# CederGroupHub/smol

Measured on AMD Instinct MI355X. Metric: attempted MC flips/s (node) + ns/flip/replica, 4096-site FCC canonical, higher is better.
Workload: dtype f64

## Files before the change

smol_amd/csrc/mc_lean.h:

```cpp
#pragma once
#include "smolmc_common.h"

template <int CTRL> __device__ __forceinline__ double dpp_xor_add(double v) {
    const int lo = __builtin_amdgcn_update_dpp(__double2loint(v), __double2loint(v), CTRL, 0xf, 0xf, true);
    const int hi = __builtin_amdgcn_update_dpp(__double2hiint(v), __double2hiint(v), CTRL, 0xf, 0xf, true);
    return v + __hiloint2double(hi, lo);
}
__device__ __forceinline__ double wave_sum_all(double v) {
    v = dpp_xor_add<0xB1>(v);
    v = dpp_xor_add<0x4E>(v);
    v = dpp_xor_add<0x141>(v);
    v = dpp_xor_add<0x140>(v);
    {
        const unsigned lo = (unsigned)__double2loint(v), hi = (unsigned)__double2hiint(v);
        const auto a = __builtin_amdgcn_permlane16_swap(lo, lo, false, false);
        const auto b = __builtin_amdgcn_permlane16_swap(hi, hi, false, false);
        v = __hiloint2double((int)b[0], (int)a[0]) + __hiloint2double((int)b[1], (int)a[1]);
    }
    {
        const unsigned lo = (unsigned)__double2loint(v), hi = (unsigned)__double2hiint(v);
        const auto a = __builtin_amdgcn_permlane32_swap(lo, lo, false, false);
        const auto b = __builtin_amdgcn_permlane32_swap(hi, hi, false, false);
        v = __hiloint2double((int)b[0], (int)a[0]) + __hiloint2double((int)b[1], (int)a[1]);
    }
    return v;
}

template <int CTRL> __device__ __forceinline__ float dpp_add_f32(float v) {
    const int t = __builtin_amdgcn_update_dpp(0, __float_as_int(v), CTRL, 0xf, 0xf, true);
    return v + __int_as_float(t);
}
__device__ __forceinline__ float wave_sum_f32_uniform(float v) {
    v = dpp_add_f32<0xB1>(v);
    v = dpp_add_f32<0x4E>(v);
    v = dpp_add_f32<0x141>(v);
    v = dpp_add_f32<0x140>(v);
    float total;
    asm volatile("s_nop 1\n\t"
                 "v_add_f32_dpp %1, %1, %1 row_bcast:15 row_mask:0xa bank_mask:0xf\n\t"
                 "s_nop 1\n\t"
                 "v_add_f32_dpp %1, %1, %1 row_bcast:31 row_mask:0xc bank_mask:0xf\n\t"
                 "s_nop 1\n\t"
                 "v_readlane_b32 %0, %1, 63\n\t"
                 "s_nop 1"
                 : "=s"(total), "+v"(v));
    return total;
}


__device__ __forceinline__ double lean_ewald_partial(const LeanParams &P, const uint8_t *occ, int lane,
                                                     int s, int swa, int swm, int swb) {
    const double *g = P.ew_G + (size_t)s * P.ew_nact;
    const int W = P.ew_W, na = P.ew_nact;
    double out = 0;
    for (int j0 = lane; j0 < na; j0 += 64 * 8) {
        int k[8];
        double gk[8], q[8];
#pragma unroll
        for (int u = 0; u < 8; ++u) {
            const int jj = min(j0 + 64 * u, na - 1);
            k[u] = P.ew_act[jj];
            gk[u] = g[jj];
        }
#pragma unroll
        for (int u = 0; u < 8; ++u)
            q[u] = P.ew_qs[(size_t)k[u] * W + (int)occ[lean_swz(k[u], swa, swm, swb)]];
#pragma unroll
        for (int u = 0; u < 8; ++u)
            out = fma((j0 + 64 * u < na && k[u] != s) ? q[u] : 0.0, gk[u], out);
    }
    return out;
}

template <int FOOT = 2, bool PRE = false>
__device__ __forceinline__ void field_apply(const LeanParams &P, double *phi, int lane, int s, double dq,
                                            const uint32_t (&e0)[27], const bool have_e0) {
    const int js = s - P.sbase;
    const double keep = phi[js];
    const LeanParamsKernarg Q = rare_params();
    const unsigned char *gx = (const unsigned char *)Q->ew_gx;
    if (gx != nullptr) {
        const uint32_t *E8 = Q->ew_E8;
        const uint32_t s8[1] = {Q->ew_S8[js]};
        const double d[1] = {dq};
        if (PRE && have_e0) field_sweep_gx_pre27(phi, E8, gx, lane, P.ew_nact, s8, d, e0);
        else field_sweep_gx_multi<1, FOOT>(phi, E8, gx, lane, P.ew_nact, s8, d);
    } else {
        const double *g = P.ew_G + (size_t)s * P.ew_nact;
        field_sweep<false>(phi, g, g, lane, P.ew_nact, dq, 0.0);
    }
    phi[js] = keep;
}

template <int FOOT = 2>
__device__ __forceinline__ void field_apply(const LeanParams &P, double *phi, int lane, int s, double dq) {
    const uint32_t none[27] = {};
    field_apply<FOOT, false>(P, phi, lane, s, dq, none, false);
}

template <int FOOT = 1, bool FEW = false>
__device__ __forceinline__ void field_apply_flips(double *phi, int lane, int nfl, int vsite, double vdq) {
    const LeanParamsKernarg Q = rare_params();

    const unsigned char *gx = (const unsigned char *)Q->ew_gx;
    auto site_of = [&](int f) { return (int)rdlane((uint32_t)vsite, f); };
    auto dq_of = [&](int f) {
        return __hiloint2double((int)rdlane((uint32_t)__double2hiint(vdq), f), (int)rdlane((uint32_t)__double2loint(vdq), f));
    };
    const int sb = Q->sbase, na = Q->ew_nact;
    if (gx == nullptr) {
        const double *G = Q->ew_G;
        for (int f = 0; f < nfl; ++f) {
            const double dqf = dq_of(f);
            if (dqf == 0.0) continue;
            const double *g = G + (size_t)site_of(f) * na;
            field_sweep<false>(phi, g, g, lane, na, dqf, 0.0);
        }
        return;
    }
    const uint32_t *E8 = Q->ew_E8, *S8 = Q->ew_S8;
    for (int f0 = 0; f0 < nfl; f0 += 4) {
        const int n = min(4, nfl - f0);
        uint32_t s8[4];
        double dq[4];
#pragma unroll
        for (int k = 0; k < 4; ++k) {
            const int f = k < n ? f0 + k : f0;
            s8[k] = S8[site_of(f) - sb];
            dq[k] = k < n ? dq_of(f) : 0.0;
        }
        if (FEW && n <= 3) {
            const uint32_t a[3] = {s8[0], s8[1], s8[2]};
            const double d[3] = {dq[0], dq[1], dq[2]};
            field_sweep_gx_multi<3, FOOT>(phi, E8, gx, lane, na, a, d);
        } else if (n == 1) {
            const uint32_t a[1] = {s8[0]};
            const double d[1] = {dq[0]};
            field_sweep_gx_multi<1, FOOT>(phi, E8, gx, lane, na, a, d);
        } else if (n == 2) {
            const uint32_t a[2] = {s8[0], s8[1]};
            const double d[2] = {dq[0], dq[1]};
            field_sweep_gx_multi<2, FOOT>(phi, E8, gx, lane, na, a, d);
        } else if (n == 3) {
            const uint32_t a[3] = {s8[0], s8[1], s8[2]};
            const double d[3] = {dq[0], dq[1], dq[2]};
            field_sweep_gx_multi<3, FOOT>(phi, E8, gx, lane, na, a, d);
        } else {
            field_sweep_gx_multi<4, FOOT>(phi, E8, gx, lane, na, s8, dq);
        }
    }
}

template <int FOOT = 1>
__device__ __forceinline__ void field_apply2(const LeanParams &P, double *phi, int lane, int s1, double dq1,
                                             int s2, double dq2) {
    const int j1 = s1 - P.sbase, j2 = s2 - P.sbase;
    const LeanParamsKernarg Q = rare_params();
    const unsigned char *gx = (const unsigned char *)Q->ew_gx;
    if (gx != nullptr) {
        const uint32_t *E8 = Q->ew_E8, *S8 = Q->ew_S8;
        const uint32_t s8[2] = {S8[j1], S8[j2]};
        const double d[2] = {dq1, dq2};
        field_sweep_gx_multi<2, FOOT>(phi, E8, gx, lane, P.ew_nact, s8, d);
        return;
    }
    const double *g1 = P.ew_G + (size_t)s1 * P.ew_nact, *g2 = P.ew_G + (size_t)s2 * P.ew_nact;
    const double keep1 = phi[j1], keep2 = phi[j2];
    const double c12 = g2[j1], c21 = g1[j2];
    field_sweep<true>(phi, g1, g2, lane, P.ew_nact, dq1, dq2);
    if (j1 != j2) {
        phi[j1] = fma(dq2, c12, keep1);
        phi[j2] = fma(dq1, c21, keep2);
    } else {
        phi[j1] = keep1;
    }
}

__device__ __forceinline__ uint32_t bounded(uint32_t a, uint32_t lim) {
#ifdef SMOLMC_BOUNDS
    if (a >= lim) __builtin_trap();
#else
    (void)lim;
#endif
    return a;
}

template <int NW> struct RowWords { uint32_t w[NW]; };
template <int NW>
__device__ __forceinline__ RowWords<NW> load_row(__amdgpu_buffer_rsrc_t rs, uint32_t voff, uint32_t soff) {
    RowWords<NW> r;
    if constexpr (NW == 2) {
        const auto v = __builtin_amdgcn_raw_buffer_load_b64(rs, voff, soff, 0);
        r.w[0] = v[0]; r.w[1] = v[1];
    } else if constexpr (NW == 3) {
        const auto v = __builtin_amdgcn_raw_buffer_load_b96(rs, voff, soff, 0);
        r.w[0] = v[0]; r.w[1] = v[1]; r.w[2] = v[2];
    } else if constexpr (NW == 4) {
        const auto v = __builtin_amdgcn_raw_buffer_load_b128(rs, voff, soff, 0);
        r.w[0] = v[0]; r.w[1] = v[1]; r.w[2] = v[2]; r.w[3] = v[3];
    } else if constexpr (NW == 6) {
        const auto v = __builtin_amdgcn_raw_buffer_load_b128(rs, voff, soff, 0);
        const auto u = __builtin_amdgcn_raw_buffer_load_b64(rs, voff + 16u, soff, 0);
        r.w[0] = v[0]; r.w[1] = v[1]; r.w[2] = v[2]; r.w[3] = v[3]; r.w[4] = u[0]; r.w[5] = u[1];
    } else {
        static_assert(NW % 4 == 0, "row width");
#pragma unroll
        for (int b = 0; b < NW / 4; ++b) {
            const auto v = __builtin_amdgcn_raw_buffer_load_b128(rs, voff + 16u * b, soff, 0);
            r.w[4 * b] = v[0]; r.w[4 * b + 1] = v[1]; r.w[4 * b + 2] = v[2]; r.w[4 * b + 3] = v[3];
        }
    }
    return r;
}
template <int NW> __device__ __forceinline__ uint32_t row_entry(const RowWords<NW> &r, int q) {
    return (r.w[q >> 1] >> (16 * (q & 1))) & 0xffffu;
}
template <bool WIDE, int NW> __device__ __forceinline__ uint32_t row_addr(const RowWords<NW> &r, int q) {
    if constexpr (WIDE) return r.w[q];
    else return row_entry<NW>(r, q);
}

__device__ __noinline__ double wl_flatness_check(const double *wl_S, long long *wl_Hh, int L, double flat,
                                                 double div, double wl_m, int lane) {
    long cnt = 0;
    double sum = 0;
    for (int i = lane; i < L; i += 64)
        if (wl_S[i] > 0) { cnt++; sum += (double)wl_Hh[i]; }
    const double tcnt = wave_sum_all((double)cnt), tsum = wave_sum_all(sum);
    if (tcnt >= 2.0) {
        const double thr = flat * (tsum / tcnt);
        int bad = 0;
        for (int i = lane; i < L; i += 64)
            if (wl_S[i] > 0 && !((double)wl_Hh[i] > thr)) bad = 1;
        if (__ballot(bad) == 0ull) {
            for (int i = lane; i < L; i += 64) wl_Hh[i] = 0;
            wl_m = wl_m / div;
        }
    }
    return wl_m;
}

__device__ __noinline__ double wl_multi_flatness_check(const double *S, uint32_t *cnt, double *occb, long long *hist_g,
                                                       long long *occ_g, int L, double flat, double div, double wl_m, int lane) {
    long n = 0;
    double sum = 0;
    for (int i = lane; i < L; i += 64)
        if (S[i] > 0) { n++; sum += (double)(hist_g[i] + (long long)cnt[i]); }
    const double tn = wave_sum_all((double)n), tsum = wave_sum_all(sum);
    if (tn >= 2.0) {
        const double thr = flat * (tsum / tn);
        int bad = 0;
        for (int i = lane; i < L; i += 64)
            if (S[i] > 0 && !((double)(hist_g[i] + (long long)cnt[i]) > thr)) bad = 1;
        if (__ballot(bad) == 0ull) {
            for (int i = lane; i < L; i += 64) {
                hist_g[i] = 0;
                occ_g[i] += (long long)cnt[i];
                if (occb) occb[i] += (double)cnt[i];
                cnt[i] = 0u;
            }
            wl_m = wl_m / div;
        }
    }
    return wl_m;
}

typedef __attribute__((address_space(3))) uint8_t lds_u8_t;
typedef __attribute__((address_space(3))) double lds_f64_t;
#if defined(__HIP_DEVICE_COMPILE__)
#define SMOLMC_LDS_U8(a) (*(lds_u8_t *)(a))
#define SMOLMC_LDS_F64(a) (*(const lds_f64_t *)(a))
#else
#define SMOLMC_LDS_U8(a) (*(uint8_t *)(uintptr_t)(a))
#define SMOLMC_LDS_F64(a) (*(const double *)(uintptr_t)(a))
#endif
template <bool ABS> __device__ __forceinline__ uint8_t occ_ld(const uint8_t *occ, uint32_t a) {
    if constexpr (ABS) return SMOLMC_LDS_U8(a);
    else return occ[a];
}
__device__ __forceinline__ uint32_t opaque_u32(uint32_t v) {
    asm volatile("" : "+s"(v));
    return v;
}
template <bool ABS> __device__ __forceinline__ void occ_st(uint8_t *occ, uint32_t a, uint8_t v) {
    if constexpr (ABS) SMOLMC_LDS_U8(a) = v;
    else occ[a] = v;
}

constexpr bool lean_rows(int MM) { return MM >= 10; }
constexpr int lean_mm_of(int MM, int it) { return !lean_rows(MM) ? MM : (it == 0 ? MM / 10 : MM % 10); }
constexpr int lean_mm_max(int MM) { return !lean_rows(MM) ? MM : (MM / 10 > MM % 10 ? MM / 10 : MM % 10); }
constexpr int lean_row_off(int MM, int it) { return !lean_rows(MM) ? it * MM : (it == 0 ? 0 : MM / 10); }
constexpr int lean_row_len(int MM, int NSLOT) { return !lean_rows(MM) ? NSLOT * MM : MM / 10 + MM % 10; }

template <int NSLOT, int MM, int STEP, bool HAS_MU, int EWX, bool WL, bool BIAS = false, bool SOLO = false,
          int KF = 0, int OCC = 0, bool REPLAY = false>
__global__ void __attribute__((amdgpu_waves_per_eu(OCC ? OCC : 1, OCC ? OCC : 8)))
__launch_bounds__(256) mc_lean_kernel(const LeanParams P) {
    static_assert(KF == 0 || (!WL && !BIAS && !SOLO), "correlation-function tables: plain Metropolis layouts only");
    static_assert(!REPLAY || (!WL && OCC == 0), "replay: Metropolis variants (Wang-Landau: mc_wl_kernel)");
    constexpr int NACC = KF ? KF : 1;
    constexpr int EWM = EWX & 3;
    constexpr bool WMU = (EWX & 4) != 0;
    static_assert(!WMU || (HAS_MU && !WL && !REPLAY), "per-walker chemical potentials: semigrand Metropolis variants");
    constexpr bool ROWS = lean_rows(MM);
    constexpr int MMX = lean_mm_max(MM);
    constexpr bool STRAIGHT = ROWS && STEP == SMOLMC_STEP_SWAP && OCC == 0 && !HAS_MU;
    static_assert(!ROWS || (SOLO && NSLOT == 2 && EWX == 0 && !REPLAY && KF == 0 && !WL && !BIAS), "solo rows: plain Metropolis, solo layout");
    constexpr bool HAS_EW = EWM != 0, ew_field = EWM == 2;
    extern __shared__ __attribute__((aligned(16))) unsigned char smem[];
    if ((uint32_t)(uintptr_t)smem != 0u) __builtin_trap();
    const int lane = threadIdx.x & 63;
    const int wave = SOLO ? 0 : threadIdx.x >> 6;
    const int nwaves = SOLO ? 1 : blockDim.x >> 6;
    const int r = uni(blockIdx.x * nwaves + wave);
    const size_t per_wave = (size_t)P.Nlds + 64 * 8 + (WL ? (size_t)P.wl.L * 24 : 0) +
                            ((HAS_EW && ew_field) ? 64 + (size_t)P.ew_nact * 8 : 0);
    double *s_dt = SOLO ? (double *)(smem + ((per_wave + 15) & ~(size_t)15)) : (double *)smem;
    const uint32_t dt_off = SOLO ? (uint32_t)((per_wave + 15) & ~(size_t)15) : 0u;
    double *s_mu = s_dt + P.dt_len;
    double *s_q = s_mu + 8, *s_dg = s_mu + 16;
    unsigned char *wbase = SOLO ? smem : (unsigned char *)(s_mu + 24) + (size_t)wave * per_wave;
    uint8_t *occ = wbase;
    double *s_feat = (double *)(wbase + P.Nlds);
    double *wl_S = s_feat + 64;
    long long *wl_Hh = (long long *)(wl_S + (WL ? P.wl.L : 0));
    long long *wl_Oc = wl_Hh + (WL ? P.wl.L : 0);
    double *phi = (double *)(wbase + P.Nlds + 64 * 8 + 64);
    const int swa = P.swz_a, swm = P.swz_m, swb = P.swz_b;
    for (int i = threadIdx.x; i < P.dt_len; i += blockDim.x) s_dt[i] = P.dt[i];
    if (HAS_MU && !WMU && threadIdx.x < 8) s_mu[threadIdx.x] = threadIdx.x < P.ncodes ? P.mu_row[threadIdx.x] : 0.0;
    if (WMU) {
        s_mu = (double *)(smem + P.mu_cell_off) + uni(wave * 8);
        if (lane < 8 && r < P.R) s_mu[lane] = lane < P.ncodes ? P.mu_row[(size_t)r * 8 + lane] : 0.0;
    }
    if (HAS_EW && ew_field && threadIdx.x < 8) {
        s_q[threadIdx.x] = P.ew_qrow[threadIdx.x];
        s_dg[threadIdx.x] = P.ew_dgrow[threadIdx.x];
    }
    const bool live = r < P.R;
    if (live) {
        const uint32_t *src = (const uint32_t *)(P.occ + (size_t)r * P.Npad);
        for (int i = lane; i < P.Npad / 4; i += 64)
            *(uint32_t *)(occ + lean_swz(4 * i, swa, swm, swb)) = src[i];
        s_feat[lane] = (WL && lane < P.F) ? P.features[(size_t)r * P.F + lane] : 0.0;
        if (HAS_EW && ew_field)
            for (int j = lane; j < P.ew_nact; j += 64) phi[j] = P.ew_phi[(size_t)r * P.ew_nact + j];
        if (WL)
            for (int i = lane; i < P.wl.L; i += 64) {
                wl_S[i] = P.wl.entropy[(size_t)r * P.wl.L + i];
                wl_Hh[i] = P.wl.hist[(size_t)r * P.wl.L + i];
                wl_Oc[i] = P.wl.occur[(size_t)r * P.wl.L + i];
            }
    }
    __syncthreads();
    if (!live) return;

    constexpr bool EPRE = HAS_EW && STEP == SMOLMC_STEP_FLIP && !REPLAY;
    uint32_t ereg[27] = {};
    bool epre_on = false;
    if (EPRE) {
        const LeanParamsKernarg Q = rare_params();
        const uint32_t *E8 = Q->ew_E8;
        epre_on = ew_field && Q->ew_gx != nullptr && (Q->ew_nact >> 6) >= 27;
        if (epre_on) {
#pragma unroll
            for (int u = 0; u < 27; ++u) ereg[u] = E8[64 * u + lane];
        }
    }

    uint32_t doff8[NSLOT], st8[NSLOT][MMX], sfeat[NSLOT];
    double wgt[NSLOT], acc[NSLOT], sfs[NSLOT];
    double accK[NSLOT][NACC];
    uint32_t kslot[NSLOT];
#pragma unroll
    for (int it = 0; it < NSLOT; ++it) {
        const LeanSlot sl = P.slots[it * 64 + lane];
        doff8[it] = sl.doff8 + dt_off;
        sfeat[it] = sl.feat;
        sfs[it] = sl.live ? sl.fs : 0.0;
        kslot[it] = sl.live;
#pragma unroll
        for (int m = 0; m < (ROWS ? lean_mm_of(MM, it) : MM); ++m) st8[it][m] = sl.stride8[m];
        wgt[it] = sl.w;
        acc[it] = 0.0;
#pragma unroll
        for (int k = 0; k < NACC; ++k) accK[it][k] = 0.0;
    }
    const int wl_stride = WL ? P.F : 64;
    const int wl_k = WL ? max(1, min(8, 63 / max(wl_stride, 1))) : 1;
    uint32_t sfeat_wl[NSLOT];
#pragma unroll
    for (int it = 0; it < NSLOT; ++it) sfeat_wl[it] = sfeat[it] + (uint32_t)((lane % wl_k) * wl_stride);
    int wl_rd[8];
#pragma unroll
    for (int k = 0; k < 8; ++k) wl_rd[k] = (WL && k < wl_k && lane < wl_stride) ? lane + k * wl_stride : 63;
    auto wl_cur_feat = [&]() -> double {
        const int f = lane < wl_stride ? lane : 0;
        double t[8];
#pragma unroll
        for (int k = 0; k < 8; ++k) t[k] = k < wl_k ? s_feat[f + (k < wl_k ? k : 0) * wl_stride] : 0.0;
        return ((t[0] + t[1]) + (t[2] + t[3])) + ((t[4] + t[5]) + (t[6] + t[7]));
    };
    auto reduce_features = [&](double *dst) {
#pragma unroll
        for (int it = 0; it < NSLOT; ++it) {
            if (KF == 0) {
                __hip_atomic_fetch_add(&dst[sfeat[it]], sfs[it] * acc[it], __ATOMIC_RELAXED,
                                       __HIP_MEMORY_SCOPE_WAVEFRONT);
            } else {
#pragma unroll
                for (int k = 0; k < NACC; ++k) {
                    const bool on = (uint32_t)k < kslot[it];
                    __hip_atomic_fetch_add(&dst[sfeat[it] + (on ? k : 0)], on ? sfs[it] * accK[it][k] : 0.0,
                                           __ATOMIC_RELAXED, __HIP_MEMORY_SCOPE_WAVEFRONT);
                }
            }
        }
    };
    double H = P.enthalpy[r];
    const double nbeta = WL ? 0.0 : -P.beta[r];
    double wl_m = WL ? P.wl.m[r] : 0.0;
    double wl_bq = WL ? floordiv_exact(H - P.wl.vmin, P.wl.bin) : 0.0;
    const double wl_inv_bin = WL ? 1.0 / P.wl.bin : 0.0;
    long long wl_counter = WL ? P.wl.counter[r] : 0;
    long long wl_rem_check = WL ? (P.wl.check ? wl_counter % P.wl.check : 1) : 0;
    unsigned long long step = P.nsteps[r];
    uint32_t nacc_add = 0;
    const uint32_t key0 = (uint32_t)P.seeds[r], key1 = (uint32_t)(P.seeds[r] >> 32);
    const uint32_t nact = (uint32_t)P.nact, nt8 = P.nt8, snt8 = P.snt8;
    const int sbase = P.sbase;
    double acc_mu = 0.0, acc_ew = 0.0;
    const int btype = BIAS ? P.bias_type : 0;
    const int brows = (btype && btype != SMOLMC_BIAS_FUGACITY) ? P.bias_rows : 0;
    double bias_acc = 0.0, chg[SMOLMC_MAX_BIAS_ROWS];
#pragma unroll
    for (int k = 0; k < SMOLMC_MAX_BIAS_ROWS; ++k) chg[k] = k < brows ? P.charge[(size_t)r * SMOLMC_MAX_BIAS_ROWS + k] : 0.0;
    constexpr bool FAST = !WL && !HAS_EW;
    float thr_lo = 0.0f, thr_hi = 0.0f;
    const double inv_nbeta = FAST ? 1.0 / nbeta : 0.0;
    uint32_t nacc_before = 0;
    int nsite = 0, naddr = 0;
    double *featp = P.features + (size_t)r * P.F;
    const double base_feat = lane < P.F ? featp[lane] : 0.0;
    uint32_t smp_countdown = P.smp.every ? (uint32_t)P.smp.every : 0xffffffffu;
    long long smp_index = 0;
    uint32_t W0 = 0;
    int cand[4] = {0, 0, 0, 0}, canda[4] = {0, 0, 0, 0};
    double vGc = 0.0;
    double logu = 0.0;
    unsigned long long batch64_base = ~0ull;
    unsigned long long batch_base = ~0ull;
    constexpr int ROW = lean_row_len(MM, NSLOT);
    constexpr int NW = SOLO ? ROW : ROW / 2;
    constexpr uint32_t ENT = SOLO ? 4u : 2u;
    constexpr uint32_t SITE_BYTES = 64u * ROW * ENT;
    const __amdgpu_buffer_rsrc_t idx_rs = __builtin_amdgcn_make_buffer_rsrc(
        SOLO ? (void *)P.idx32 : (void *)P.idx, 0, 0x7fffffff, 0x00020000);
    const uint32_t lane_voff = (uint32_t)lane * (ROW * ENT);

    int s1, a1;
    RowWords<NW> row1;
    uint32_t ridx = 0;
    double lu_rp = 0.0;
    int rp_bad = 0;
    auto rp_site = [&](const uint32_t i) -> int {
        const int v = uni(P.rp_steps[((size_t)r * (uint32_t)P.steps + i) * 4]);
        return v >= 0 ? v : sbase;
    };
    {
        if (REPLAY) {
            s1 = rp_site(0u);
        } else {
            const unsigned long long sp = step - 1ull;
            const uint32_t w = (uint32_t)uni((int)philox4x32_10((uint32_t)sp, (uint32_t)(sp >> 32), 0u, 0u,
                                                                key0, key1).w[1]);
            s1 = sbase + (int)__umulhi(w, nact);
        }
        a1 = lean_swz(s1, swa, swm, swb);
        row1 = load_row<NW>(idx_rs, lane_voff, (uint32_t)(ROWS ? a1 : s1) * SITE_BYTES);
    }

    double *wl_pend = WL ? P.wl.meanf + (size_t)r * P.wl.L * P.F : nullptr;
    double wl_pc[8] = {0.0, 0.0, 0.0, 0.0, 0.0, 0.0, 0.0, 0.0};
    auto wl_pend_sum = [&]() -> double {
        return ((wl_pc[0] + wl_pc[1]) + (wl_pc[2] + wl_pc[3])) + ((wl_pc[4] + wl_pc[5]) + (wl_pc[6] + wl_pc[7]));
    };
    uint32_t steps_left = (uint32_t)P.steps;
    while (steps_left != 0u) {
        const unsigned long long base = step & ~15ull;
        if (!REPLAY && base != batch_base) {
            batch_base = base;
            const unsigned long long st = base + (unsigned)(lane >> 2);
            const philox_out o = philox4x32_10((uint32_t)st, (uint32_t)(st >> 32), (uint32_t)(lane & 3),
                                               0u, key0, key1);
            W0 = o.w[0];
            nsite = sbase + (int)__umulhi(o.w[1], nact);
            naddr = lean_swz(nsite, swa, swm, swb);
            if ((step & ~63ull) != batch64_base) {
                batch64_base = step & ~63ull;
                const unsigned long long s64 = batch64_base + (unsigned)lane;
                const philox_out a = philox4x32_10((uint32_t)s64, (uint32_t)(s64 >> 32), 0u, 0u, key0, key1);
                logu = log(philox_u53(a.w[2], a.w[3]));
                if (FAST) {
                    const double thr = logu * inv_nbeta;
                    const double eps = P.fast_eps + 1e-6 * fabs(thr);
                    thr_lo = P.fast_eps > 0.0 ? (float)(thr - eps) : -INFINITY;
                    thr_hi = P.fast_eps > 0.0 ? (float)(thr + eps) : INFINITY;
                }
            }
            if (STEP == SMOLMC_STEP_SWAP) {
                cand[0] = sbase + (int)__umulhi(o.w[0], nact);
                cand[1] = sbase + (int)__umulhi(o.w[1], nact);
                cand[2] = sbase + (int)__umulhi(o.w[2], nact);
                cand[3] = sbase + (int)__umulhi(o.w[3], nact);
#pragma unroll
                for (int j = 0; j < 4; ++j) canda[j] = lean_swz(cand[j], swa, swm, swb);
                if (HAS_EW && ew_field) {
                    const int prev = __shfl(nsite, (lane & ~3) - 4);
                    const int site_l = lane < 4 ? s1 : prev;
                    vGc = P.ew_G[(size_t)cand[0] * P.ew_nact + (site_l - sbase)];
                }
            }
        }
        uint32_t chunk = 16u - (uint32_t)(step & 15ull);
        chunk = min(chunk, steps_left);
        chunk = min(chunk, smp_countdown);
        steps_left -= chunk;
        smp_countdown -= chunk;
        const unsigned long long chunk_end = step + chunk;
        int l4 = (int)(step & 15ull) * 4;
        int l64 = (int)(step & 63ull);
        do {
        __builtin_amdgcn_s_setprio(1);
        int s1n, a1n;
        int rq1 = 0, rq2 = -1, rq3 = 0;
        bool rp_empty = false;
        if (REPLAY) {
            const int *rec = P.rp_steps + ((size_t)r * (uint32_t)P.steps + ridx) * 4;
            const int q0 = uni(rec[0]);
            rq1 = uni(rec[1]); rq2 = uni(rec[2]); rq3 = uni(rec[3]);
            rp_empty = q0 < 0;
            double u = uni_d(P.rp_u[(size_t)r * (uint32_t)P.steps + ridx]);
            if (u != u) u = 0.0;
            lu_rp = log(u);
            s1n = ridx + 1u < (uint32_t)P.steps ? rp_site(ridx + 1u) : s1;
            a1n = lean_swz(s1n, swa, swm, swb);
            if (FAST) {
                const double thr = lu_rp * inv_nbeta, eps = P.fast_eps + 1e-6 * fabs(thr);
                thr_lo = P.fast_eps > 0.0 ? (float)(thr - eps) : -INFINITY;
                thr_hi = P.fast_eps > 0.0 ? (float)(thr + eps) : INFINITY;
            }
        } else {
            s1n = (int)rdlane((uint32_t)nsite, l4);
            a1n = (int)rdlane((uint32_t)naddr, l4);
        }
        uint32_t va1 = (uint32_t)a1;
        asm volatile("" : "+v"(va1));
        const int vo1 = (int)occ_ld<SOLO>(occ, va1);
        const int o1 = uni(vo1);
        int nfl, s2, a2, n1, n2 = 0, o2 = 0;
        if (STEP != SMOLMC_STEP_SWAP) { s2 = s1; a2 = a1; }
        int fb = -1;
        if (REPLAY) {
            if (STEP == SMOLMC_STEP_FLIP) {
                nfl = rp_empty ? 0 : 1;
                n1 = rp_empty ? o1 : rq1;
                rp_bad |= (rq2 >= 0) ? 1 : 0;
            } else if (!rp_empty && rq2 >= 0) {
                nfl = 2;
                s2 = rq2;
                a2 = lean_swz(s2, swa, swm, swb);
                o2 = uni((int)occ_ld<SOLO>(occ, (uint32_t)a2));
                n2 = rq3;
                n1 = rq1;
                rp_bad |= (n2 != o1 || n1 != o2) ? 1 : 0;
                n2 = o1; n1 = o2;
            } else {
                nfl = 0; s2 = s1; a2 = a1; o2 = o1; n2 = o1; n1 = o1;
                rp_bad |= (!rp_empty || rq2 >= 0) ? 1 : 0;
            }
        } else if (STEP == SMOLMC_STEP_FLIP) {
            const uint32_t kk = __umulhi(rdlane(W0, l4 + 1), (uint32_t)(P.ncodes - 1));
            n1 = (int)kk + ((int)kk >= o1 ? 1 : 0);
            nfl = 1;
        } else {
            nfl = 2;
            n2 = o1;
#define SMOLMC_CAND_MASK(J)                                                                        \
    const int v##J = (int)occ_ld<SOLO>(occ, (uint32_t)canda[J]);                                   \
    const unsigned long long m##J = __ballot(v##J != o1) & (0xEull << l4);
#define SMOLMC_CAND_TAKE(J)                                                                        \
    {                                                                                              \
        const int b = __ffsll((long long)m##J) - 1;                                                \
        s2 = (int)rdlane((uint32_t)cand[J], b);                                                    \
        a2 = (int)rdlane((uint32_t)canda[J], b);                                                   \
        o2 = (int)rdlane((uint32_t)v##J, b);                                                       \
        if (J == 0) fb = b;                                                                        \
    }
            SMOLMC_CAND_MASK(0)
            if constexpr (STRAIGHT) {
                unsigned long long mt = m0;
                uint32_t ta = (uint32_t)canda[0];
                int tv = v0;
                if (__builtin_expect(m0 == 0ull, 0)) {
                    SMOLMC_CAND_MASK(1)
                    mt = m1; ta = (uint32_t)canda[1]; tv = v1;
                    if (m1 == 0ull) {
                        SMOLMC_CAND_MASK(2)
                        mt = m2; ta = (uint32_t)canda[2]; tv = v2;
                        if (m2 == 0ull) {
                            SMOLMC_CAND_MASK(3)
                            mt = m3; ta = (uint32_t)canda[3]; tv = v3;
                            if (m3 == 0ull) {
                                mt = 1ull; ta = va1; tv = o1; nfl = 0;
                                const unsigned long long cur = chunk_end - chunk;
                                for (uint32_t q = 0;; ++q) {
                                    const philox_out o = philox4x32_10((uint32_t)cur, (uint32_t)(cur >> 32),
                                                                       4u + 64u * q + (uint32_t)lane, 0u, key0, key1);
                                    int selsite = -1, selv = 0;
#pragma unroll
                                    for (int j = 3; j >= 0; --j) {
                                        const int cs = sbase + (int)__umulhi(o.w[j], nact);
                                        const int v = (int)occ[lean_swz(cs, swa, swm, swb)];
                                        if (v != o1) { selsite = lean_swz(cs, swa, swm, swb); selv = v; }
                                    }
                                    const unsigned long long m = __ballot(selsite >= 0);
                                    if (m) {
                                        const int b = __ffsll((long long)m) - 1;
                                        ta = rdlane((uint32_t)selsite, b);
                                        tv = (int)rdlane((uint32_t)selv, b);
                                        nfl = 2;
                                        break;
                                    }
                                    if ((q & 63u) == 0) {
                                        int any = 0;
                                        for (uint32_t a = lane; a < nact; a += 64)
                                            any |= ((int)occ[lean_swz(sbase + (int)a, swa, swm, swb)] != o1);
                                        if (__ballot(any) == 0ull) break;
                                    }
                                }
                            }
                        }
                    }
                }
                const int b = __ffsll((long long)mt) - 1;
                a2 = (int)rdlane(ta, b);
                o2 = (int)rdlane((uint32_t)tv, b);
                s2 = a2;
            } else
            if (m0) SMOLMC_CAND_TAKE(0)
            else {
                SMOLMC_CAND_MASK(1)
                if (m1) SMOLMC_CAND_TAKE(1)
                else {
                    SMOLMC_CAND_MASK(2)
                    if (m2) SMOLMC_CAND_TAKE(2)
                    else {
                        SMOLMC_CAND_MASK(3)
                        if (m3) SMOLMC_CAND_TAKE(3)
                        else {
                            bool hit = false;
                            const unsigned long long cur = chunk_end - chunk;
                            for (uint32_t q = 0;; ++q) {
                                const philox_out o = philox4x32_10((uint32_t)cur, (uint32_t)(cur >> 32),
                                                                   4u + 64u * q + (uint32_t)lane, 0u, key0, key1);
                                int selsite = -1, selv = 0;
#pragma unroll
                                for (int j = 3; j >= 0; --j) {
                                    const int cs = sbase + (int)__umulhi(o.w[j], nact);
                                    const int v = (int)occ[lean_swz(cs, swa, swm, swb)];
                                    if (v != o1) { selsite = ROWS ? lean_swz(cs, swa, swm, swb) : cs; selv = v; }
                                }
                                const unsigned long long m = __ballot(selsite >= 0);
                                if (m) {
                                    const int b = __ffsll((long long)m) - 1;
                                    s2 = (int)rdlane((uint32_t)selsite, b);
                                    a2 = ROWS ? s2 : lean_swz(s2, swa, swm, swb);
                                    o2 = (int)rdlane((uint32_t)selv, b);
                                    hit = true;
                                    break;
                                }
                                if ((q & 63u) == 0) {
                                    int any = 0;
                                    for (uint32_t a = lane; a < nact; a += 64)
                                        any |= ((int)occ[lean_swz(sbase + (int)a, swa, swm, swb)] != o1);
                                    if (__ballot(any) == 0ull) break;
                                }
                            }
                            if (!hit) { nfl = 0; s2 = s1; a2 = a1; o2 = o1; }
                        }
                    }
                }
            }
#undef SMOLMC_CAND_MASK
#undef SMOLMC_CAND_TAKE
            n1 = o2;
        }

        __builtin_amdgcn_s_setprio(2);
        RowWords<NW> row2 = row1;
        if (STEP == SMOLMC_STEP_SWAP) {
            row2 = load_row<NW>(idx_rs, lane_voff, (uint32_t)(ROWS ? a2 : s2) * SITE_BYTES);
        }
        if (WL) {
            unsafeAtomicAdd(wl_pend + lane, wl_pend_sum());
        }

        constexpr bool DIFF = STEP == SMOLMC_STEP_SWAP;
        double e = 0.0, d1[NSLOT], d2[NSLOT];
        uint32_t dp[NSLOT];
        uint32_t ad1[NSLOT], ad2[NSLOT];
        {
            const uint32_t pair1 = (uint32_t)o1 * snt8 + (uint32_t)n1 * nt8;
#pragma unroll
            for (int it = 0; it < NSLOT; ++it) {
                uint32_t a = doff8[it];
                if (DIFF) a = dp[it] = doff8[it] + pair1;
#pragma unroll
                for (int m = 0; m < (ROWS ? lean_mm_of(MM, it) : MM); ++m) a += __umul24(st8[it][m], (uint32_t)occ_ld<SOLO>(occ, bounded(row_addr<SOLO, NW>(row1, (ROWS ? lean_row_off(MM, it) : it * MM) + m), (uint32_t)P.Nlds)));
                if (DIFF) {
                    d1[it] = SMOLMC_LDS_F64(a);
                    if (KF) ad1[it] = a;
                } else {
                    d1[it] = SMOLMC_LDS_F64(a + pair1);
                    if (KF) ad1[it] = a + pair1;
                    e = fma(wgt[it], d1[it], e);
                }
            }
        }
        row1 = load_row<NW>(idx_rs, lane_voff, (uint32_t)(ROWS ? a1n : s1n) * SITE_BYTES);
        double ew_part = 0.0, ew_uni = 0.0;
        double dq1 = 0.0, dq2 = 0.0;
        if (HAS_EW) {
            if (ew_field) {
                dq1 = s_q[n1] - s_q[o1];
                ew_uni = 2.0 * dq1 * phi[s1 - sbase] + (s_dg[n1] - s_dg[o1]);
            } else {
                const int W = P.ew_W;
                dq1 = P.ew_qs[(size_t)s1 * W + n1] - P.ew_qs[(size_t)s1 * W + o1];
                ew_part = 2.0 * dq1 * lean_ewald_partial(P, occ, lane, s1, swa, swm, swb);
                ew_uni = 2.0 * dq1 * P.ew_frozen[s1] +
                         (P.ew_dg[(size_t)s1 * W + n1] - P.ew_dg[(size_t)s1 * W + o1]);
            }
        }
        if (STEP == SMOLMC_STEP_SWAP) {
            occ_st<SOLO>(occ, va1, (uint8_t)n1);
            const uint32_t pair2 = (uint32_t)o2 * snt8 + (uint32_t)n2 * nt8;
#pragma unroll
            for (int it = 0; it < NSLOT; ++it) {
                uint32_t a = DIFF ? dp[it] : doff8[it];
#pragma unroll
                for (int m = 0; m < (ROWS ? lean_mm_of(MM, it) : MM); ++m) a += __umul24(st8[it][m], (uint32_t)occ_ld<SOLO>(occ, bounded(row_addr<SOLO, NW>(row2, (ROWS ? lean_row_off(MM, it) : it * MM) + m), (uint32_t)P.Nlds)));
                if (DIFF) {
                    d1[it] -= SMOLMC_LDS_F64(a);
                    if (KF) ad2[it] = a;
                    e = fma(wgt[it], d1[it], e);
                } else {
                    d2[it] = SMOLMC_LDS_F64(a + pair2);
                    if (KF) ad2[it] = a + pair2;
                    e = fma(wgt[it], d2[it], e);
                }
            }
            if (HAS_EW) {
                if (ew_field) {
                    dq2 = s_q[n2] - s_q[o2];
                    const double cross =
                        fb >= 0 ? __hiloint2double((int)rdlane((uint32_t)__double2hiint(vGc), fb),
                                                   (int)rdlane((uint32_t)__double2loint(vGc), fb))
                                : P.ew_G[(size_t)s2 * P.ew_nact + (s1 - sbase)];
                    ew_uni += 2.0 * dq2 * (phi[s2 - sbase] + dq1 * cross) + (s_dg[n2] - s_dg[o2]);
                } else {
                    const int W = P.ew_W;
                    dq2 = P.ew_qs[(size_t)s2 * W + n2] - P.ew_qs[(size_t)s2 * W + o2];
                    ew_part += 2.0 * dq2 * lean_ewald_partial(P, occ, lane, s2, swa, swm, swb);
                    ew_uni += 2.0 * dq2 * P.ew_frozen[s2] +
                              (P.ew_dg[(size_t)s2 * W + n2] - P.ew_dg[(size_t)s2 * W + o2]);
                }
            }
        }
        double dMu = 0.0;
        if (HAS_MU && nfl >= 1) {
            dMu = s_mu[n1] - s_mu[o1];
            if (nfl == 2) dMu += s_mu[n2] - s_mu[o2];
        }
        double dH = 0.0, dEw = 0.0;
        double wl_nbq = 0.0;
        double dB = 0.0, dQ[SMOLMC_MAX_BIAS_ROWS] = {0.0, 0.0, 0.0, 0.0};
        if (btype && nfl >= 1) {
            if (btype == SMOLMC_BIAS_FUGACITY) {
                dB = P.bias_pair[o1 * 8 + n1];
                if (nfl == 2) dB += P.bias_pair[o2 * 8 + n2];
            } else {
                double sq_new = 0.0, sq_old = 0.0;
#pragma unroll
                for (int k = 0; k < SMOLMC_MAX_BIAS_ROWS; ++k)
                    if (k < brows) {
                        const double *bp = P.bias_pair + k * P.bias_row_stride;
                        double x = bp[o1 * 8 + n1];
                        if (nfl == 2) x += bp[o2 * 8 + n2];
                        dQ[k] = x;
                        const double cn = chg[k] + x;
                        sq_old += chg[k] * chg[k];
                        sq_new += cn * cn;
                    }
                dB = -P.bias_pen * sq_new - (-P.bias_pen * sq_old);
            }
        }
        auto exact_decision = [&]() -> bool {
            dH = wave_sum_all(e);
            if (HAS_EW) {
                dEw = (ew_field ? 0.0 : wave_sum_all(ew_part)) + ew_uni;
                dH += P.ew_coef * dEw;
            }
            if (HAS_MU) dH -= dMu;
            const double lu = REPLAY ? lu_rp
                                     : __hiloint2double((int)rdlane((uint32_t)__double2hiint(logu), l64),
                                                        (int)rdlane((uint32_t)__double2loint(logu), l64));
            if (!WL) {
                const double exponent = nbeta * dH + 0.0 + dB;
                return __ballot((exponent >= 0.0) || (exponent > lu)) != 0ull;
            } else {
                const double new_h = H + dH;
                if (new_h < P.wl.vmin || new_h >= P.wl.vmax) {
                    return false;
                } else {
                    const int b = (int)wl_bq;
                    wl_nbq = floordiv_exact_inv(new_h - P.wl.vmin, P.wl.bin, wl_inv_bin);
                    const int nb = (int)wl_nbq;
                    const double exponent = wl_S[b] - wl_S[nb] + 0.0;
                    return __ballot((exponent >= 0.0) || (exponent > lu)) != 0ull;
                }
            }
        };
        constexpr bool SELACC = DIFF && FAST && !BIAS;
        uint32_t sel_hi = 0u;
        auto on_accept = [&]() {
            if (KF) {
                const unsigned char *kb = (const unsigned char *)P.dtk;
#pragma unroll
                for (int it = 0; it < NSLOT; ++it) {
                    const uint32_t g1 = doff8[it] * (uint32_t)(SMOLMC_LEAN_MAX_KF - 1) + ad1[it];
                    const uint32_t g2 = doff8[it] * (uint32_t)(SMOLMC_LEAN_MAX_KF - 1) + ad2[it];
#pragma unroll
                    for (int k = 0; k < NACC; ++k) {
                        const bool on = (uint32_t)k < kslot[it];
                        const uint32_t off = (uint32_t)k * P.ktab8;
                        double v = on ? *(const double *)(kb + (g1 + off)) : 0.0;
                        if (STEP == SMOLMC_STEP_SWAP) {
                            const double v2 = on ? *(const double *)(kb + (g2 + off)) : 0.0;
                            v = DIFF ? v - v2 : v + v2;
                        }
                        accK[it][k] += v;
                    }
                }
            }
            if (SELACC) {
                sel_hi = 0x3ff00000u;
            } else if (!WL) {
#pragma unroll
                for (int it = 0; it < NSLOT; ++it) acc[it] += d1[it];
                if (STEP == SMOLMC_STEP_SWAP && !DIFF) {
#pragma unroll
                    for (int it = 0; it < NSLOT; ++it) acc[it] += d2[it];
                }
            } else {
#pragma unroll
                for (int it = 0; it < NSLOT; ++it) {
                    const double dd = (STEP == SMOLMC_STEP_SWAP && !DIFF) ? d1[it] + d2[it] : d1[it];
                    __hip_atomic_fetch_add(&s_feat[sfeat_wl[it]], sfs[it] * dd, __ATOMIC_RELAXED,
                                           __HIP_MEMORY_SCOPE_WAVEFRONT);
                }
            }
            if (STEP == SMOLMC_STEP_FLIP) occ_st<SOLO>(occ, va1, (uint8_t)n1);
            if (STEP == SMOLMC_STEP_SWAP) occ_st<SOLO>(occ, (uint32_t)a2, (uint8_t)(ROWS ? vo1 : n2));
            if (HAS_EW && ew_field) {
                if (STEP == SMOLMC_STEP_SWAP) {
                    if (dq1 != 0.0 || dq2 != 0.0) field_apply2(P, phi, lane, s1, dq1, s2, dq2);
                } else if (dq1 != 0.0) {
                    field_apply<2, EPRE>(P, phi, lane, s1, dq1, ereg, epre_on);
                }
            }
            acc_mu += dMu;
            acc_ew += dEw;
            bias_acc += dB;
#pragma unroll
            for (int k = 0; k < SMOLMC_MAX_BIAS_ROWS; ++k) chg[k] += dQ[k];
            if (!FAST) H += dH;
            if (!SELACC) nacc_add++;
        };
        auto on_reject = [&]() {
            if (STEP == SMOLMC_STEP_SWAP) {
            occ_st<SOLO>(occ, va1, (uint8_t)(ROWS ? vo1 : o1));
            }
        };
        nacc_before = nacc_add;
        bool accepted = false;
        __builtin_amdgcn_s_setprio(3);
        if (FAST && !BIAS) {
            const float ef = (float)((HAS_MU && lane == 0) ? e - dMu : e);
            const float S = wave_sum_f32_uniform(ef);
            const unsigned long long bit = 1ull << (REPLAY ? 0 : l64);
            const bool ca = (__ballot(S < thr_lo) & bit) != 0ull;
            const bool cr = (__ballot(S > thr_hi) & bit) != 0ull;
            if constexpr (STRAIGHT) {
                bool ok = ca;
                if (__builtin_expect(!(ca || cr), 0)) ok = exact_decision();
                sel_hi = ok ? 0x3ff00000u : 0u;
                uint32_t vst = (uint32_t)vo1;
                asm("" : "+v"(vst));
                occ_st<SOLO>(occ, ok ? (uint32_t)a2 : va1, (uint8_t)vst);
            } else
            if (ca) on_accept();
            else if (cr) on_reject();
            else if (exact_decision()) on_accept();
            else on_reject();
        } else {
            accepted = exact_decision();
            if (accepted) on_accept();
            else on_reject();
        }
        if (SELACC) {
            const uint32_t sh = (uint32_t)uni((int)sel_hi);
            const double sel = __hiloint2double((int)sh, 0);
#pragma unroll
            for (int it = 0; it < NSLOT; ++it) acc[it] = fma(sel, d1[it], acc[it]);
            nacc_add += sh >> 29;
        }
        s1 = s1n;
        a1 = a1n;
        __builtin_amdgcn_s_setprio(0);
        if (REPLAY) {
            double lane_e = 0.0;
            if (FAST) {
#pragma unroll
                for (int it = 0; it < NSLOT; ++it) lane_e = fma(wgt[it], acc[it], lane_e);
            }
            const double Hnow = FAST ? H + (wave_sum_all(lane_e) - acc_mu) : H;
            if (lane == 0) {
                const size_t k = (size_t)r * (uint32_t)P.steps + ridx;
                P.rp_acc[k] = (uint8_t)(nacc_add != nacc_before);
                P.rp_H[k] = Hnow;
            }
            ridx++;
        }

        if (WL) {
            const double bq = accepted ? wl_nbq : wl_bq;
            wl_bq = bq;
            if (bq >= 0.0 && bq < (double)P.wl.L) {
                const int b = (int)bq;
                wl_counter++;
                if (++wl_rem_check == P.wl.check) wl_rem_check = 0;
                wl_pend = P.wl.meanf + ((size_t)r * P.wl.L + b) * P.F;
#pragma unroll
                for (int k = 0; k < 8; ++k) wl_pc[k] = s_feat[wl_rd[k]];
                if (lane == 0) {
                    __hip_atomic_fetch_add(&wl_S[b], wl_m, __ATOMIC_RELAXED, __HIP_MEMORY_SCOPE_WAVEFRONT);
                    __hip_atomic_fetch_add(&wl_Hh[b], 1ll, __ATOMIC_RELAXED, __HIP_MEMORY_SCOPE_WAVEFRONT);
                    __hip_atomic_fetch_add(&wl_Oc[b], 1ll, __ATOMIC_RELAXED, __HIP_MEMORY_SCOPE_WAVEFRONT);
                }
            }
            if (wl_rem_check == 0) {
                const LeanParamsKernarg Q = rare_params();
                wl_m = wl_flatness_check(wl_S, wl_Hh, Q->wl.L, Q->wl.flat, Q->wl.div, wl_m, lane);
            }
        }

        l4 += 4;
        l64 += 1;
        } while (--chunk != 0u);
        step = chunk_end;

        if (smp_countdown == 0) {
            const LeanParamsKernarg Q = rare_params();
            const int qF = Q->F, qFce = Q->Fce;
            double *const q_feat = Q->smp.feat;
            smp_countdown = (uint32_t)Q->smp.every;
            const size_t row = (size_t)smp_index * Q->R + r;
            smp_index++;
            if (WL) {
                const double fcur = wl_cur_feat();
                if (lane < qF) q_feat[row * qF + lane] = fcur;
            } else {
                s_feat[lane] = 0.0;
                reduce_features(s_feat);
                if (lane < qFce) q_feat[row * qF + lane] = base_feat + s_feat[lane];
            }
            if (!WL && HAS_EW && lane == qFce) q_feat[row * qF + lane] = base_feat + acc_ew;
            if (!WL && HAS_MU && lane == qFce + (HAS_EW ? 1 : 0))
                q_feat[row * qF + lane] = base_feat + acc_mu;
            double lane_e = 0.0;
            if (FAST) {
#pragma unroll
                for (int it = 0; it < NSLOT; ++it) lane_e = fma(wgt[it], acc[it], lane_e);
            }
            const double Hnow = FAST ? H + (wave_sum_all(lane_e) - acc_mu) : H;
            if (lane == 0) {
                Q->smp.H[row] = Hnow;
                Q->smp.acc[row] = (uint8_t)(nacc_add != nacc_before);
                if (BIAS && Q->smp_bias_off) (Q->smp.H + Q->smp_bias_off)[row] = Q->bias[r] + bias_acc;
            }
            if (Q->smp.occ) {
                const int qNpad = Q->Npad;
                uint32_t *dst = (uint32_t *)(Q->smp.occ + row * qNpad);
                for (int i = lane; i < qNpad / 4; i += 64)
                    dst[i] = *(const uint32_t *)(occ + lean_swz(4 * i, swa, swm, swb));
            }
        }
    }

    if (HAS_EW && ew_field)
        for (int j = lane; j < P.ew_nact; j += 64) P.ew_phi[(size_t)r * P.ew_nact + j] = phi[j];
    {
        uint32_t *dst = (uint32_t *)(P.occ + (size_t)r * P.Npad);
        for (int i = lane; i < P.Npad / 4; i += 64)
            dst[i] = *(const uint32_t *)(occ + lean_swz(4 * i, swa, swm, swb));
    }
    if (WL) {
        const double fcur = wl_cur_feat();
        unsafeAtomicAdd(wl_pend + lane, wl_pend_sum());
        if (lane < P.F) featp[lane] = fcur;
        for (int i = lane; i < P.wl.L; i += 64) {
            P.wl.entropy[(size_t)r * P.wl.L + i] = wl_S[i];
            P.wl.hist[(size_t)r * P.wl.L + i] = wl_Hh[i];
            P.wl.occur[(size_t)r * P.wl.L + i] = wl_Oc[i];
        }
        if (lane == 0) {
            P.wl.m[r] = wl_m;
            P.wl.counter[r] = wl_counter;
        }
    } else {
        s_feat[lane] = 0.0;
        reduce_features(s_feat);
        if (lane < P.Fce) featp[lane] = base_feat + s_feat[lane];
    }
    if (FAST) {
        double lane_e = 0.0;
#pragma unroll
        for (int it = 0; it < NSLOT; ++it) lane_e = fma(wgt[it], acc[it], lane_e);
        H += wave_sum_all(lane_e) - acc_mu;
    }
    if (btype && lane == 0) {
        P.bias[r] += bias_acc;
#pragma unroll
        for (int k = 0; k < SMOLMC_MAX_BIAS_ROWS; ++k)
            if (k < brows) P.charge[(size_t)r * SMOLMC_MAX_BIAS_ROWS + k] = chg[k];
    }
    if (REPLAY && lane == 0 && rp_bad) atomicOr(P.rp_err, 1);
    if (lane == 0) {
        if (!WL && HAS_EW) featp[P.Fce] += acc_ew;
        if (!WL && HAS_MU) featp[P.Fce + (HAS_EW ? 1 : 0)] += acc_mu;
        P.enthalpy[r] = H;
        P.nsteps[r] = step;
        P.nacc[r] += nacc_add;
        if (P.steps) P.last_acc[r] = (uint8_t)(nacc_add != nacc_before);
    }
}


__device__ __noinline__ philox_out philox_call(uint32_t c0, uint32_t c1, uint32_t c2, uint32_t k0, uint32_t k1) {
    return philox4x32_10(c0, c1, c2, 0u, k0, k1);
}

__device__ __forceinline__ double table_log_count_ratio(const double *lnt, int u, int n0, int nc) {
    const int au = u < 0 ? -u : u;
    const int sgn = u < 0 ? -1 : 1;
    const int first = u < 0 ? n0 : n0 + 1;
    double t[4];
#pragma unroll
    for (int k = 0; k < 4; ++k) t[k] = k < au ? lnt[first + sgn * k] : 0.0;
    double part = 0.0;
#pragma unroll
    for (int k = 0; k < 4; ++k) part += t[k];
    for (int k = 4; k < au; ++k) part += lnt[first + sgn * k];
    part = u < 0 ? part : -part;
    double tot = 0.0;
    for (int c = 0; c < nc; ++c)
        tot += __hiloint2double((int)rdlane((uint32_t)__double2hiint(part), c),
                                (int)rdlane((uint32_t)__double2loint(part), c));
    return tot;
}

__device__ __noinline__ void wl_multi_row_swap(double *grows, double *crow, int old_bin, int new_bin, int F, int lane, int sum_mode);

template <int NSLOT, int MM, int EWX, bool REPLAY = false, bool BIAS = false, bool WLT = false>
__global__ void __launch_bounds__(512) mc_table_kernel(const LeanParams P) {
    constexpr int EWM = EWX & 3;
    constexpr bool WMU = (EWX & 4) != 0;
    static_assert(!WMU || (!WLT && !REPLAY), "per-walker chemical potentials: semigrand Metropolis variants");
    static_assert(!(WLT && BIAS), "Cannot apply bias to Wang-Landau simulation (wanglandau.py:127-128)");
    static_assert(!(WLT && REPLAY), "Wang-Landau TableFlip replays take the universal kernel");
    constexpr bool has_ew = EWM != 0, ew_field = EWM == 2;
    extern __shared__ __attribute__((aligned(16))) unsigned char smem[];
    const int lane = threadIdx.x & 63;
    const int wave = threadIdx.x >> 6;
    const int nwaves = blockDim.x >> 6;
    const int slot = uni(blockIdx.x * nwaves + wave);
    const int r = (P.order != nullptr && slot < P.R) ? uni(P.order[slot]) : slot;
    double *s_dt = (double *)smem;
    double *s_mu = s_dt + P.dt_len;
    const size_t per_wave = (size_t)P.Nlds + 64 * 8 + 64 + (ew_field ? (size_t)P.ew_nact * 8 : 0) +
                            (WLT ? wl_multi_wave_bytes(P.wl.L, P.F, P.wl.sum_mode) : 0);
    double *s_q = s_mu + 8, *s_dg = s_mu + 16;
    double *s_tfw = s_mu + 24;
    int *s_tf = (int *)(s_tfw + 16);
    double *s_ln = s_tfw + 16 + 32;
    unsigned char *wbase = (unsigned char *)(s_ln + P.tf_ln_len) + (size_t)wave * per_wave;
    uint8_t *occ = wbase;
    double *s_feat = (double *)(wbase + P.Nlds);
    int *s_cnt = (int *)(s_feat + 64);
    double *phi = (double *)(wbase + P.Nlds + 64 * 8 + 64);
    const int wl_sum_mode = WLT ? P.wl.sum_mode : 1;
    double *wl_S = phi + (ew_field ? P.ew_nact : 0);
    uint32_t *wl_cnt = (uint32_t *)(wl_S + (WLT ? P.wl.L : 0));
    double *wl_occb = (double *)((unsigned char *)wl_cnt + (WLT ? (((size_t)P.wl.L * 4 + 7) & ~(size_t)7) : 0));
    double *s_rows = wl_occb + ((WLT && !wl_sum_mode) ? P.wl.L : 0);
    const int swa = P.swz_a, swm = P.swz_m, swb = P.swz_b;
    const bool has_mu = P.mu_row != nullptr;
    for (int i = threadIdx.x; i < P.dt_len; i += blockDim.x) s_dt[i] = P.dt[i];
    if (!WMU && threadIdx.x < 8) s_mu[threadIdx.x] = (has_mu && threadIdx.x < P.ncodes) ? P.mu_row[threadIdx.x] : 0.0;
    if (WMU) {
        s_mu = (double *)(smem + P.mu_cell_off) + uni(wave * 8);
        if (lane < 8 && r < P.R) s_mu[lane] = lane < P.ncodes ? P.mu_row[(size_t)r * 8 + lane] : 0.0;
// ... 1054 lines not shown
```

Before: 19.02 billion.

## Branchless accept path with per-lane thresholds and early loop-counter advance in straight swap kernel

For the STRAIGHT swap variant, the accept decision now reads the per-step thresholds into a lane before the reduction, leaves the wave sum in lane 63 without a readlane, and tests sign bits of the upper ballot half. The result is turned into a mask that drives a branchless occupancy store and accept counter. For MM==21 it also issues the second-row LDS gathers first and advances the loop counters and l64 inside the tail, adjusting the logu lane index to match. The aim is to shorten the serial scalar/vector dependency chain at the end of each step, at the cost of more fragile scheduling and index bookkeeping.

Result: faster. 20.15 billion (median of 6 runs) (+5.9%).

```diff
diff --git a/smol_amd/csrc/mc_lean.h b/smol_amd/csrc/mc_lean.h
--- a/smol_amd/csrc/mc_lean.h
+++ b/smol_amd/csrc/mc_lean.h
@@ -46,7 +46,18 @@
                  : "=s"(total), "+v"(v));
     return total;
 }
-
+__device__ __forceinline__ float wave_sum_f32_lane63(float v) {
+    v = dpp_add_f32<0xB1>(v);
+    v = dpp_add_f32<0x4E>(v);
+    v = dpp_add_f32<0x141>(v);
+    v = dpp_add_f32<0x140>(v);
+    asm volatile("s_nop 1\n\t"
+                 "v_add_f32_dpp %0, %0, %0 row_bcast:15 row_mask:0xa bank_mask:0xf\n\t"
+                 "s_nop 1\n\t"
+                 "v_add_f32_dpp %0, %0, %0 row_bcast:31 row_mask:0xc bank_mask:0xf"
+                 : "+v"(v));
+    return v;
+}
 
 __device__ __forceinline__ double lean_ewald_partial(const LeanParams &P, const uint8_t *occ, int lane,
                                                      int s, int swa, int swm, int swb) {
@@ -306,6 +317,7 @@
     constexpr bool ROWS = lean_rows(MM);
     constexpr int MMX = lean_mm_max(MM);
     constexpr bool STRAIGHT = ROWS && STEP == SMOLMC_STEP_SWAP && OCC == 0 && !HAS_MU;
+    constexpr int TAIL_AHEAD = (STRAIGHT && MM == 21) ? 1 : 0;
     static_assert(!ROWS || (SOLO && NSLOT == 2 && EWX == 0 && !REPLAY && KF == 0 && !WL && !BIAS), "solo rows: plain Metropolis, solo layout");
     constexpr bool HAS_EW = EWM != 0, ew_field = EWM == 2;
     extern __shared__ __attribute__((aligned(16))) unsigned char smem[];
@@ -531,6 +543,8 @@
         const unsigned long long chunk_end = step + chunk;
         int l4 = (int)(step & 15ull) * 4;
         int l64 = (int)(step & 63ull);
+        float tlo_s = 0.0f, thi_s = 0.0f;
+        uint32_t va2 = 0u, okm = 0u;
         do {
         __builtin_amdgcn_s_setprio(1);
         int s1n, a1n;
@@ -554,6 +568,10 @@
         } else {
             s1n = (int)rdlane((uint32_t)nsite, l4);
             a1n = (int)rdlane((uint32_t)naddr, l4);
+        }
+        if constexpr (STRAIGHT) {
+            tlo_s = __uint_as_float(rdlane(__float_as_uint(thr_lo), l64));
+            thi_s = __uint_as_float(rdlane(__float_as_uint(thr_hi), l64));
         }
         uint32_t va1 = (uint32_t)a1;
         asm volatile("" : "+v"(va1));
@@ -747,6 +765,29 @@
         if (STEP == SMOLMC_STEP_SWAP) {
             occ_st<SOLO>(occ, va1, (uint8_t)n1);
             const uint32_t pair2 = (uint32_t)o2 * snt8 + (uint32_t)n2 * nt8;
+            if constexpr (TAIL_AHEAD != 0) {
+                uint32_t g[NSLOT][MMX];
+#pragma unroll
+                for (int it = 0; it < NSLOT; ++it) {
+#pragma unroll
+                    for (int m = 0; m < lean_mm_of(MM, it); ++m) g[it][m] = (uint32_t)occ_ld<SOLO>(occ, bounded(row_addr<SOLO, NW>(row2, lean_row_off(MM, it) + m), (uint32_t)P.Nlds));
+                }
+                __builtin_amdgcn_sched_barrier(0);
+                l4 = (int)opaque_u32((uint32_t)l4 + 4u);
+                l64 = (int)opaque_u32((uint32_t)l64 + 1u);
+                chunk = opaque_u32(chunk - 1u);
+                va2 = (uint32_t)a2;
+                asm volatile("" : "+v"(va2));
+                __builtin_amdgcn_sched_barrier(0);
+#pragma unroll
+                for (int it = 0; it < NSLOT; ++it) {
+                    uint32_t a = dp[it];
+#pragma unroll
+                    for (int m = 0; m < lean_mm_of(MM, it); ++m) a += __umul24(st8[it][m], g[it][m]);
+                    d1[it] -= SMOLMC_LDS_F64(a);
+                    e = fma(wgt[it], d1[it], e);
+                }
+            } else
 #pragma unroll
             for (int it = 0; it < NSLOT; ++it) {
                 uint32_t a = DIFF ? dp[it] : doff8[it];
@@ -815,8 +856,8 @@
             }
             if (HAS_MU) dH -= dMu;
             const double lu = REPLAY ? lu_rp
-                                     : __hiloint2double((int)rdlane((uint32_t)__double2hiint(logu), l64),
-                                                        (int)rdlane((uint32_t)__double2loint(logu), l64));
+                                     : __hiloint2double((int)rdlane((uint32_t)__double2hiint(logu), l64 - TAIL_AHEAD),
+                                                        (int)rdlane((uint32_t)__double2loint(logu), l64 - TAIL_AHEAD));
             if (!WL) {
                 const double exponent = nbeta * dH + 0.0 + dB;
                 return __ballot((exponent >= 0.0) || (exponent > lu)) != 0ull;
@@ -899,22 +940,28 @@
         __builtin_amdgcn_s_setprio(3);
         if (FAST && !BIAS) {
             const float ef = (float)((HAS_MU && lane == 0) ? e - dMu : e);
+            if constexpr (STRAIGHT) {
+                const float Sv = wave_sum_f32_lane63(ef);
+                const uint32_t ha = opaque_u32((uint32_t)(__ballot(Sv < tlo_s) >> 32));
+                const uint32_t hr = opaque_u32((uint32_t)(__ballot(Sv > thi_s) >> 32));
+                okm = (uint32_t)((int)ha >> 31);
+                if (__builtin_expect((int)(ha | hr) >= 0, 0)) okm = 0u - (uint32_t)uni((int)exact_decision());
+                okm = opaque_u32(okm);
+                sel_hi = okm & 0x3ff00000u;
+                uint32_t vst = (uint32_t)vo1;
+                asm("" : "+v"(vst));
+                const uint32_t vb = TAIL_AHEAD ? va2 : (uint32_t)a2;
+                occ_st<SOLO>(occ, (vb & okm) | (va1 & ~okm), (uint8_t)vst);
+            } else {
             const float S = wave_sum_f32_uniform(ef);
             const unsigned long long bit = 1ull << (REPLAY ? 0 : l64);
             const bool ca = (__ballot(S < thr_lo) & bit) != 0ull;
             const bool cr = (__ballot(S > thr_hi) & bit) != 0ull;
-            if constexpr (STRAIGHT) {
-                bool ok = ca;
-                if (__builtin_expect(!(ca || cr), 0)) ok = exact_decision();
-                sel_hi = ok ? 0x3ff00000u : 0u;
-                uint32_t vst = (uint32_t)vo1;
-                asm("" : "+v"(vst));
-                occ_st<SOLO>(occ, ok ? (uint32_t)a2 : va1, (uint8_t)vst);
-            } else
             if (ca) on_accept();
             else if (cr) on_reject();
             else if (exact_decision()) on_accept();
             else on_reject();
+            }
         } else {
             accepted = exact_decision();
             if (accepted) on_accept();
@@ -925,6 +972,8 @@
             const double sel = __hiloint2double((int)sh, 0);
 #pragma unroll
             for (int it = 0; it < NSLOT; ++it) acc[it] = fma(sel, d1[it], acc[it]);
+            if constexpr (STRAIGHT) nacc_add -= okm;
+            else
             nacc_add += sh >> 29;
         }
         s1 = s1n;
@@ -967,9 +1016,12 @@
             }
         }
 
+        if constexpr (!TAIL_AHEAD) {
         l4 += 4;
         l64 += 1;
-        } while (--chunk != 0u);
+        --chunk;
+        }
+        } while (chunk != 0u);
         step = chunk_end;
 
         if (smp_countdown == 0) {
```
